# henreedev/audio-pathtracer

Hardware: NVIDIA B200
Metric: bdpt_path_pairs_per_second (higher is better)
Workload: dtype f32 + u64 Q32.32

## Files before the change

audio-pathtracer_b200/csrc/fs_bvh_build.cu:

```cuda
#include "fs_internal.h"
#include <vector>
#include <utility>
#include <stdlib.h>

namespace {

__device__ __forceinline__ uint32_t f2ord(float f)
{
    uint32_t u = __float_as_uint(f);
    return (u & 0x80000000u) ? ~u : (u | 0x80000000u);
}
__host__ __device__ __forceinline__ float ord2f(uint32_t u)
{
    u = (u & 0x80000000u) ? (u & 0x7fffffffu) : ~u;
#if defined(__CUDA_ARCH__)
    return __uint_as_float(u);
#else
    float f; memcpy(&f, &u, 4); return f;
#endif
}

__global__ void k_init_bounds(uint32_t* bounds)
{
    if (threadIdx.x < 3) bounds[threadIdx.x] = 0xffffffffu;
// ... 642 lines not shown
            const int r = c[pick].ref;
            load_children(nodes, r, c[pick], c[k]);
            ++k;
        }
    }
    float lx = c[0].lx, hx = c[0].hx, ly = c[0].ly, hy = c[0].hy, lz = c[0].lz, hz = c[0].hz;
    for (int j = 1; j < k; ++j) {
        lx = fminf(lx, c[j].lx); hx = fmaxf(hx, c[j].hx); ly = fminf(ly, c[j].ly); hy = fmaxf(hy, c[j].hy);
        lz = fminf(lz, c[j].lz); hz = fmaxf(hz, c[j].hz);
    }
    if (!(hx < 1e29f) || !(lx > -1e29f) || !(hy < 1e29f) || !(hz < 1e29f)) {
        hx = fminf(hx, 1e29f); hy = fminf(hy, 1e29f); hz = fminf(hz, 1e29f);
    }
    const float mx = 0.5f * (lx + hx), my = 0.5f * (ly + hy), mz = 0.5f * (lz + hz);
    int slot_of[8], child_in[8];
    for (int j = 0; j < 8; ++j) { slot_of[j] = -1; child_in[j] = -1; }
    for (int it = 0; it < k; ++it) {
        float best = -3.0e38f; int bc = -1, bs = -1;
        for (int j = 0; j < k; ++j) {
            if (slot_of[j] >= 0) continue;
            const float dx = 0.5f * (c[j].lx + c[j].hx) - mx, dy = 0.5f * (c[j].ly + c[j].hy) - my, dz = 0.5f * (c[j].lz + c[j].hz) - mz;
            for (int s = 0; s < 8; ++s) {
                if (child_in[s] >= 0) continue;
                const float cost = ((s & 1) ? dx : -dx) + ((s & 2) ? dy : -dy) + ((s & 4) ? dz : -dz);
                if (cost > best) { best = cost; bc = j; bs = s; }
            }
        }
        slot_of[bc] = bs; child_in[bs] = bc;
    }
    const int ebx = q8_exponent(hx - lx), eby = q8_exponent(hy - ly), ebz = q8_exponent(hz - lz);
    const float ix = __uint_as_float((uint32_t)(254 - ebx) << 23), iy = __uint_as_float((uint32_t)(254 - eby) << 23),
                iz = __uint_as_float((uint32_t)(254 - ebz) << 23);
    uint32_t q[12];
    for (int w = 0; w < 12; ++w) q[w] = 0u;
    uint32_t imask = 0, lmask = 0;
    int refs[8];
    for (int s = 0; s < 8; ++s) {
        const int j = child_in[s];
        uint32_t b[6];
        if (j < 0) { b[0] = b[1] = b[2] = 255u; b[3] = b[4] = b[5] = 0u; refs[s] = W8_EMPTY; }
        else {
            b[0] = q8_lo(c[j].lx, lx, ix); b[1] = q8_lo(c[j].ly, ly, iy); b[2] = q8_lo(c[j].lz, lz, iz);
            b[3] = q8_hi(c[j].hx, lx, ix); b[4] = q8_hi(c[j].hy, ly, iy); b[5] = q8_hi(c[j].hz, lz, iz);
            refs[s] = c[j].ref;
            if (c[j].ref >= 0) imask |= 1u << s; else lmask |= 1u << s;
        }
        for (int a = 0; a < 6; ++a) q[a * 2 + (s >> 2)] |= b[a] << (8 * (s & 3));
    }
    uint4* o = w8tmp + (size_t)i * 5;
    o[0] = make_uint4(__float_as_uint(lx), __float_as_uint(ly), __float_as_uint(lz), ((uint32_t)ebx << 23) | imask | (lmask << 8));
    o[1] = make_uint4((uint32_t)eby << 23, (uint32_t)ebz << 23, 0u, 0u);
    o[2] = make_uint4(q[0], q[1], q[2], q[3]);
    o[3] = make_uint4(q[4], q[5], q[6], q[7]);
    o[4] = make_uint4(q[8], q[9], q[10], q[11]);
    for (int s = 0; s < 8; ++s) w8ref[(size_t)i * 8 + s] = refs[s];
}

__global__ void k_w8_count(const uint4* __restrict__ w8tmp, const int* __restrict__ frontier, uint32_t nf,
                           uint32_t* __restrict__ cnt_in, uint32_t* __restrict__ cnt_leaf)
{
    const uint32_t t = blockIdx.x * blockDim.x + threadIdx.x;
    if (t >= nf) return;
    const uint32_t w = w8tmp[(size_t)frontier[t] * 5].w;
    cnt_in[t] = (uint32_t)__popc(w & 0xffu);
    cnt_leaf[t] = (uint32_t)__popc((w >> 8) & 0xffu);
}

__global__ void k_w8_place(const uint4* __restrict__ w8tmp, const int* __restrict__ w8ref, uint4* __restrict__ dst,
                           const int* __restrict__ frontier, uint32_t nf, const uint32_t* __restrict__ off_in,
                           const uint32_t* __restrict__ off_leaf, uint32_t level_base, uint32_t tri_level_base,
                           int* __restrict__ next_frontier, const float4* __restrict__ tris, float4* __restrict__ tris8,
                           uint32_t* __restrict__ tri8_map)
{
    const uint32_t t = blockIdx.x * blockDim.x + threadIdx.x;
    if (t >= nf) return;
    const int src = frontier[t];
    const uint4* p = w8tmp + (size_t)src * 5;
    uint4* q = dst + (size_t)(level_base + t) * 5;
    uint4 u1 = p[1];
    uint32_t oi = off_in[t], ol = tri_level_base + off_leaf[t];
    u1.z = level_base + nf + oi;
    u1.w = ol;
    q[0] = p[0]; q[1] = u1; q[2] = p[2]; q[3] = p[3]; q[4] = p[4];
    for (int s = 0; s < 8; ++s) {
        const int r = w8ref[(size_t)src * 8 + s];
        if (r == W8_EMPTY) continue;
        if (r >= 0) next_frontier[oi++] = r;
        else {
            const uint32_t first = (uint32_t)(~r) >> 3;
            for (int a = 0; a < 4; ++a) tris8[(size_t)ol * 4 + a] = tris[(size_t)first * 4 + a];
            tri8_map[ol] = first;
            ++ol;
        }
    }
}

__device__ __forceinline__ void store_children(float4* __restrict__ nodes, int i, const cbox& a, const cbox& b)
{
    nodes[(size_t)i * 4] = make_float4(a.lx, a.hx, a.ly, a.hy);
    nodes[(size_t)i * 4 + 1] = make_float4(b.lx, b.hx, b.ly, b.hy);
    nodes[(size_t)i * 4 + 2] = make_float4(a.lz, a.hz, b.lz, b.hz);
    nodes[(size_t)i * 4 + 3] = make_float4(__int_as_float(a.ref), __int_as_float(b.ref), 0.f, 0.f);
}
__device__ __forceinline__ cbox cbox_union(const cbox& a, const cbox& b, int ref)
{
    cbox u;
    u.lx = fminf(a.lx, b.lx); u.hx = fmaxf(a.hx, b.hx); u.ly = fminf(a.ly, b.ly); u.hy = fmaxf(a.hy, b.hy);
    u.lz = fminf(a.lz, b.lz); u.hz = fmaxf(a.hz, b.hz); u.ref = ref; u.src = -1;
    return u;
}

__global__ void k_bvh2_count(const float4* __restrict__ nodes, const int* __restrict__ frontier, uint32_t nf, uint32_t* __restrict__ cnt)
{
    const uint32_t t = blockIdx.x * blockDim.x + threadIdx.x;
    if (t >= nf) return;
    const float4 n3 = nodes[(size_t)frontier[t] * 4 + 3];
    cnt[t] = (__float_as_int(n3.x) >= 0 ? 1u : 0u) + (__float_as_int(n3.y) >= 0 ? 1u : 0u);
}
__global__ void k_bvh2_place(const float4* __restrict__ nodes, const int* __restrict__ frontier, uint32_t nf,
                             const uint32_t* __restrict__ off, int* __restrict__ next)
{
    const uint32_t t = blockIdx.x * blockDim.x + threadIdx.x;
    if (t >= nf) return;
    const float4 n3 = nodes[(size_t)frontier[t] * 4 + 3];
    uint32_t o = off[t];
    const int c0 = __float_as_int(n3.x), c1 = __float_as_int(n3.y);
    if (c0 >= 0) next[o++] = c0;
    if (c1 >= 0) next[o] = c1;
}

__global__ void k_rotate(float4* __restrict__ nodes, const int* __restrict__ level, uint32_t nl, uint32_t* __restrict__ n_done)
{
    const uint32_t t = blockIdx.x * blockDim.x + threadIdx.x;
    if (t >= nl) return;
    const int N = level[t];
    cbox L, R;
    load_children(nodes, N, L, R);
    float best = 0.0f; int op = 0;
    cbox LL, LR, RL, RR;
    if (R.ref >= 0) {
        load_children(nodes, R.ref, RL, RR);
        const float aR = cbox_area(R);
        const float d1 = cbox_area(cbox_union(L, RR, 0)) - aR;
        const float d2 = cbox_area(cbox_union(RL, L, 0)) - aR;
        if (d1 < best) { best = d1; op = 1; }
        if (d2 < best) { best = d2; op = 2; }
    }
    if (L.ref >= 0) {
        load_children(nodes, L.ref, LL, LR);
        const float aL = cbox_area(L);
        const float d3 = cbox_area(cbox_union(R, LR, 0)) - aL;
        const float d4 = cbox_area(cbox_union(LL, R, 0)) - aL;
        if (d3 < best) { best = d3; op = 3; }
        if (d4 < best) { best = d4; op = 4; }
    }
    if (op == 0) return;
    if (op == 1) {
        const cbox Rn = cbox_union(L, RR, R.ref);
        store_children(nodes, R.ref, L, RR);
        store_children(nodes, N, RL, Rn);
    } else if (op == 2) {
        const cbox Rn = cbox_union(RL, L, R.ref);
        store_children(nodes, R.ref, RL, L);
        store_children(nodes, N, RR, Rn);
    } else if (op == 3) {
        const cbox Ln = cbox_union(R, LR, L.ref);
        store_children(nodes, L.ref, R, LR);
        store_children(nodes, N, Ln, LL);
    } else {
        const cbox Ln = cbox_union(LL, R, L.ref);
        store_children(nodes, L.ref, LL, R);
        store_children(nodes, N, Ln, LR);
    }
    atomicAdd(n_done, 1u);
}

__global__ void k_sah_cost(uint32_t n_inner, const float4* __restrict__ nodes, double* __restrict__ out)
{
    const uint32_t i = blockIdx.x * blockDim.x + threadIdx.x;
    double a = 0.0;
    if (i < n_inner) {
        cbox c0, c1;
        load_children(nodes, (int)i, c0, c1);
        a = (double)cbox_area(c0) + (double)cbox_area(c1);
    }
    for (int o = 16; o; o >>= 1) a += __shfl_xor_sync(0xffffffffu, a, o);
    if ((threadIdx.x & 31) == 0 && a != 0.0) atomicAdd(out, a);
}

__device__ __forceinline__ void emit_single(float4 l0, float4 h0, float4* __restrict__ nodes)
{
    float pad = box_pad(l0, h0);
    const float F = 1e30f;
    nodes[0] = make_float4(l0.x - pad, h0.x + pad, l0.y - pad, h0.y + pad);
    nodes[1] = make_float4(F, F, F, F);
    nodes[2] = make_float4(l0.z - pad, h0.z + pad, F, F);
    nodes[3] = make_float4(__int_as_float(~0), __int_as_float(~0), 0.f, 0.f);
}
__global__ void k_emit_single(const float4* __restrict__ bb_lo, const float4* __restrict__ bb_hi,
                              float4* __restrict__ nodes)
{
    emit_single(bb_lo[0], bb_hi[0], nodes);
}

__global__ void k_top_treelet(const float4* __restrict__ nodes, uint32_t n_inner, uint32_t cap,
                              float4* __restrict__ top, uint32_t* __restrict__ n_top_out, int* __restrict__ queue)
{
    if (threadIdx.x != 0 || blockIdx.x != 0) return;
    uint32_t qn = 0;
    queue[qn++] = 0;
    for (uint32_t p = 0; p < qn; ++p) {
        const float4* src = nodes + (size_t)queue[p] * 4;
        float4 n3 = src[3];
        int c0 = __float_as_int(n3.x), c1 = __float_as_int(n3.y);
        if (c0 >= 0 && qn < cap) { queue[qn] = c0; c0 = FS_TOP_FLAG | (int)qn; ++qn; }
        if (c1 >= 0 && qn < cap) { queue[qn] = c1; c1 = FS_TOP_FLAG | (int)qn; ++qn; }
        top[(size_t)p * 4 + 0] = src[0];
        top[(size_t)p * 4 + 1] = src[1];
        top[(size_t)p * 4 + 2] = src[2];
        top[(size_t)p * 4 + 3] = make_float4(__int_as_float(c0), __int_as_float(c1), 0.f, 0.f);
    }
    *n_top_out = qn;
    (void)n_inner;
}

__global__ void k_leaf_stats(int n, const int2* __restrict__ ranges, uint32_t* __restrict__ max_leaf, int leaf_max)
{
    int i = blockIdx.x * blockDim.x + threadIdx.x;
    if (i >= n - 1) return;
    int cnt = ranges[i].y - ranges[i].x + 1;
    if (cnt <= leaf_max) atomicMax(max_leaf, (uint32_t)cnt);
}

__global__ void k_refit_tris(uint32_t n, const float* __restrict__ verts, const uint32_t* __restrict__ tri_orig,
                             const uint32_t* __restrict__ tri_mat, float4* __restrict__ tris, float4* __restrict__ tri_nm)
{
    const uint32_t j = blockIdx.x * blockDim.x + threadIdx.x;
    if (j >= n) return;
    pack_tri(verts, tri_orig[j], tri_mat[j], j, tris, tri_nm);
}

__device__ __forceinline__ void refit_child(int r, const float* __restrict__ verts, const uint32_t* __restrict__ tri_orig,
                                            const float4* ubox, float4& lo, float4& hi)
{
    if (r >= 0) { lo = __ldcg(ubox + 2 * (size_t)r); hi = __ldcg(ubox + 2 * (size_t)r + 1); return; }
    const uint32_t e = (uint32_t)~r, first = e >> 3, cnt = (e & 7u) + 1u;
    tri_box(verts + (size_t)tri_orig[first] * 9, lo, hi);
    for (uint32_t k = 1; k < cnt; ++k) {
        float4 l, h;
        tri_box(verts + (size_t)tri_orig[first + k] * 9, l, h);
        lo = make_float4(fminf(lo.x, l.x), fminf(lo.y, l.y), fminf(lo.z, l.z), 0.f);
        hi = make_float4(fmaxf(hi.x, h.x), fmaxf(hi.y, h.y), fmaxf(hi.z, h.z), 0.f);
    }
}

__global__ void k_refit_nodes(uint32_t n_inner, const float* __restrict__ verts, const uint32_t* __restrict__ tri_orig,
                              const int* __restrict__ parent, const uint32_t* __restrict__ need, uint32_t* __restrict__ arrive,
                              float4* __restrict__ nodes, float4* ubox)
{
    const uint32_t i = blockIdx.x * blockDim.x + threadIdx.x;
    if (i >= n_inner || need[i] != 0u) return;
    int n = (int)i;
    for (;;) {
        const float4 n3 = nodes[(size_t)n * 4 + 3];
        float4 l0, h0, l1, h1;
        refit_child(__float_as_int(n3.x), verts, tri_orig, ubox, l0, h0);
        refit_child(__float_as_int(n3.y), verts, tri_orig, ubox, l1, h1);
        const float p0 = box_pad(l0, h0), p1 = box_pad(l1, h1);
        nodes[(size_t)n * 4 + 0] = make_float4(l0.x - p0, h0.x + p0, l0.y - p0, h0.y + p0);
        nodes[(size_t)n * 4 + 1] = make_float4(l1.x - p1, h1.x + p1, l1.y - p1, h1.y + p1);
        nodes[(size_t)n * 4 + 2] = make_float4(l0.z - p0, h0.z + p0, l1.z - p1, h1.z + p1);
        __stcg(ubox + 2 * (size_t)n, make_float4(fminf(l0.x, l1.x), fminf(l0.y, l1.y), fminf(l0.z, l1.z), 0.f));
        __stcg(ubox + 2 * (size_t)n + 1, make_float4(fmaxf(h0.x, h1.x), fmaxf(h0.y, h1.y), fmaxf(h0.z, h1.z), 0.f));
        __threadfence();
        const int p = parent[n];
        if (p < 0) break;
        if (atomicAdd(arrive + p, 1u) + 1u < need[p]) break;
        __threadfence();
        n = p;
    }
}

__global__ void k_refit_single(const float* __restrict__ verts, const uint32_t* __restrict__ tri_orig, float4* __restrict__ nodes)
{
    float4 lo, hi;
    tri_box(verts + (size_t)tri_orig[0] * 9, lo, hi);
    emit_single(lo, hi, nodes);
}

__global__ void k_requant4(uint32_t n_slots, const float4* __restrict__ nodes, const int* __restrict__ wsrc,
                           const float* __restrict__ grid, uint4* __restrict__ wnodes)
{
    const uint32_t s = blockIdx.x * blockDim.x + threadIdx.x;
    if (s >= n_slots) return;
    const int src = wsrc[s];
    if (src < 0) return;
    cbox a, b;
    load_children(nodes, src >> 1, a, b);
    const cbox& c = (src & 1) ? b : a;
    const uint4 q = quant_box(c.lx, c.hx, c.ly, c.hy, c.lz, c.hz, 0, grid);
    uint4 u = wnodes[s];
    u.x = q.x; u.y = q.y; u.z = q.z;
    wnodes[s] = u;
}

}



#define BCHECK(x) do { cudaError_t e_ = (x); if (e_ != cudaSuccess) { err = e_; goto fail; } } while (0)

static void scan_u32(cudaStream_t st, const uint32_t* in, uint32_t* out, uint32_t n, uint32_t* tile_sums,
                     uint32_t* total, uint64_t* launches)
{
    const uint32_t tiles = (n + SCAN_TILE - 1) / SCAN_TILE;
    k_scan_tiles<<<tiles, SCAN_TILE, 0, st>>>(in, out, n, tile_sums);
    k_sort_scan<<<1, 1024, 0, st>>>(tile_sums, tiles);
    k_scan_add<<<tiles, SCAN_TILE, 0, st>>>(out, n, tile_sums);
    k_scan_total<<<1, 32, 0, st>>>(in, out, n, total);
    *launches += 4;
}

static cudaError_t ploc_build(cudaStream_t st, uint32_t n, const float4* bb_lo, const float4* bb_hi, float4* nodes,
                              uint64_t* launches, int radius)
{
    cudaError_t err = cudaSuccess;
    float4 *lo[2] = {nullptr, nullptr}, *hi[2] = {nullptr, nullptr};
    int* ref[2] = {nullptr, nullptr};
    uint32_t *nn = nullptr, *keep = nullptr, *mflag = nullptr, *keep_scan = nullptr, *merge_scan = nullptr,
             *tile_sums = nullptr, *totals = nullptr;
    const uint32_t n_inner = n - 1;
    const int TPB = 256;
    uint32_t cur = n, made = 0;
    int pp = 0;
    for (int k = 0; k < 2; ++k) {
        BCHECK(cudaMalloc(&lo[k], sizeof(float4) * n));
        BCHECK(cudaMalloc(&hi[k], sizeof(float4) * n));
        BCHECK(cudaMalloc(&ref[k], sizeof(int) * n));
    }
    BCHECK(cudaMalloc(&nn, 4ull * n)); BCHECK(cudaMalloc(&keep, 4ull * n)); BCHECK(cudaMalloc(&mflag, 4ull * n));
    BCHECK(cudaMalloc(&keep_scan, 4ull * n)); BCHECK(cudaMalloc(&merge_scan, 4ull * n));
    BCHECK(cudaMalloc(&tile_sums, 4ull * ((n + SCAN_TILE - 1) / SCAN_TILE + 2)));
    BCHECK(cudaMalloc(&totals, 4 * 2));
    k_ploc_init<<<(n + TPB - 1) / TPB, TPB, 0, st>>>(n, bb_lo, bb_hi, lo[0], hi[0], ref[0]); ++*launches;
    for (int round = 0; cur > 1 && round < 4096; ++round) {
        const uint32_t g = (cur + TPB - 1) / TPB;
        k_ploc_nn<<<g, TPB, 0, st>>>(cur, lo[pp], hi[pp], nn, radius);
        k_ploc_flags<<<g, TPB, 0, st>>>(cur, nn, keep, mflag);
        *launches += 2;
        scan_u32(st, keep, keep_scan, cur, tile_sums, totals, launches);
        scan_u32(st, mflag, merge_scan, cur, tile_sums, totals + 1, launches);
        k_ploc_merge<<<g, TPB, 0, st>>>(cur, nn, keep_scan, merge_scan, keep, mflag, made, n_inner, lo[pp], hi[pp], ref[pp],
                                        lo[pp ^ 1], hi[pp ^ 1], ref[pp ^ 1], nodes);
        ++*launches;
        uint32_t h[2];
        BCHECK(cudaMemcpyAsync(h, totals, sizeof(h), cudaMemcpyDeviceToHost, st));
        BCHECK(cudaStreamSynchronize(st));
        if (h[1] == 0 || h[0] >= cur) { err = cudaErrorUnknown; goto fail; }
        made += h[1];
        cur = h[0];
        pp ^= 1;
    }
    if (cur != 1 || made != n_inner) err = cudaErrorUnknown;
fail:
    for (int k = 0; k < 2; ++k) { cudaFree(lo[k]); cudaFree(hi[k]); cudaFree(ref[k]); }
    cudaFree(nn); cudaFree(keep); cudaFree(mflag); cudaFree(keep_scan); cudaFree(merge_scan); cudaFree(tile_sums); cudaFree(totals);
    return err;
}

static cudaError_t bvh2_rotate(cudaStream_t st, uint32_t n_inner, float4* nodes, int sweeps, uint64_t* launches, uint32_t* n_rot)
{
    cudaError_t err = cudaSuccess;
    int* order = nullptr;
    uint32_t *cnt = nullptr, *off = nullptr, *tile_sums = nullptr, *total = nullptr, *d_done = nullptr;
    const int TPB = 256;
    std::vector<std::pair<uint32_t, uint32_t>> levels;
    const int zero = 0;
    *n_rot = 0;
    BCHECK(cudaMalloc(&order, 4ull * n_inner));
    BCHECK(cudaMalloc(&cnt, 4ull * n_inner)); BCHECK(cudaMalloc(&off, 4ull * n_inner));
    BCHECK(cudaMalloc(&tile_sums, 4ull * ((n_inner + SCAN_TILE - 1) / SCAN_TILE + 2)));
    BCHECK(cudaMalloc(&total, 4)); BCHECK(cudaMalloc(&d_done, 4));
    BCHECK(cudaMemsetAsync(d_done, 0, 4, st));
    for (int sw = 0; sw < sweeps; ++sw) {
        levels.clear();
        BCHECK(cudaMemcpyAsync(order, &zero, 4, cudaMemcpyHostToDevice, st));
        uint32_t base = 0, nf = 1;
        while (nf) {
            levels.push_back(std::make_pair(base, nf));
            const uint32_t g = (nf + TPB - 1) / TPB;
            uint32_t next = 0;
            k_bvh2_count<<<g, TPB, 0, st>>>(nodes, order + base, nf, cnt); ++*launches;
            scan_u32(st, cnt, off, nf, tile_sums, total, launches);
            BCHECK(cudaMemcpyAsync(&next, total, 4, cudaMemcpyDeviceToHost, st));
            BCHECK(cudaStreamSynchronize(st));
            if (base + nf + next > n_inner) { err = cudaErrorUnknown; goto fail; }
            if (next) { k_bvh2_place<<<g, TPB, 0, st>>>(nodes, order + base, nf, off, order + base + nf); ++*launches; }
            base += nf; nf = next;
        }
        for (size_t l = levels.size(); l-- > 0;) {
            const uint32_t nl = levels[l].second;
            k_rotate<<<(nl + TPB - 1) / TPB, TPB, 0, st>>>(nodes, order + levels[l].first, nl, d_done); ++*launches;
        }
    }
    BCHECK(cudaMemcpyAsync(n_rot, d_done, 4, cudaMemcpyDeviceToHost, st));
    BCHECK(cudaStreamSynchronize(st));
    BCHECK(cudaGetLastError());
fail:
    cudaFree(order); cudaFree(cnt); cudaFree(off); cudaFree(tile_sums); cudaFree(total); cudaFree(d_done);
    return err;
}

static cudaError_t wide_compact(cudaStream_t st, uint32_t n_inner, const uint4* sparse, const int* sparse_prov, uint4** dense_out,
                                int** dense_prov_out, uint32_t* n_wide_out, uint64_t* launches)
{
    cudaError_t err = cudaSuccess;
    int* fr[2] = {nullptr, nullptr};
    uint32_t *cnt = nullptr, *off = nullptr, *tile_sums = nullptr, *total = nullptr;
    uint4* dense = nullptr;
    int* dense_prov = nullptr;
    const int TPB = 256;
    uint32_t nf = 1, base = 0;
    int pp = 0;
    const int zero = 0;
    BCHECK(cudaMalloc(&fr[0], 4ull * n_inner)); BCHECK(cudaMalloc(&fr[1], 4ull * n_inner));
    BCHECK(cudaMalloc(&cnt, 4ull * n_inner)); BCHECK(cudaMalloc(&off, 4ull * n_inner));
    BCHECK(cudaMalloc(&tile_sums, 4ull * ((n_inner + SCAN_TILE - 1) / SCAN_TILE + 2)));
    BCHECK(cudaMalloc(&total, 4));
    BCHECK(cudaMalloc(&dense, sizeof(uint4) * 4ull * n_inner));
    BCHECK(cudaMalloc(&dense_prov, sizeof(int) * 4ull * n_inner));
    BCHECK(cudaMemcpyAsync(fr[0], &zero, 4, cudaMemcpyHostToDevice, st));
    while (nf) {
        const uint32_t g = (nf + TPB - 1) / TPB;
        uint32_t next = 0;
        k_wide_count<<<g, TPB, 0, st>>>(sparse, fr[pp], nf, cnt); ++*launches;
        scan_u32(st, cnt, off, nf, tile_sums, total, launches);
        k_wide_place<<<g, TPB, 0, st>>>(sparse, dense, sparse_prov, dense_prov, fr[pp], nf, off, base, fr[pp ^ 1]); ++*launches;
        BCHECK(cudaMemcpyAsync(&next, total, 4, cudaMemcpyDeviceToHost, st));
        BCHECK(cudaStreamSynchronize(st));
        base += nf; nf = next; pp ^= 1;
        if (base + nf > n_inner) { err = cudaErrorUnknown; goto fail; }
    }
    BCHECK(cudaGetLastError());
    *dense_out = dense; dense = nullptr; *dense_prov_out = dense_prov; dense_prov = nullptr; *n_wide_out = base;
fail:
    cudaFree(fr[0]); cudaFree(fr[1]); cudaFree(cnt); cudaFree(off); cudaFree(tile_sums); cudaFree(total); cudaFree(dense); cudaFree(dense_prov);
    return err;
}

static cudaError_t w8_build(cudaStream_t st, uint32_t n, uint32_t n_inner, const float4* nodes, const float4* tris,
                            fs_bvh_device* out, uint64_t* launches, bool dp)
{
    cudaError_t err = cudaSuccess;
    float* T = nullptr; int* parent = nullptr; uint32_t *need = nullptr, *arrive = nullptr;
    uint4 *tmp = nullptr, *dense = nullptr, *fit = nullptr;
    int *ref = nullptr, *fr[2] = {nullptr, nullptr};
    uint32_t *cnt_in = nullptr, *cnt_leaf = nullptr, *off_in = nullptr, *off_leaf = nullptr, *tile_sums = nullptr, *total = nullptr;
    float4* tris8 = nullptr; uint32_t* map = nullptr;
    const int TPB = 256;
    uint32_t nf = 1, base = 0, tri_base = 0;
    int pp = 0;
    const int zero = 0;
    BCHECK(cudaMalloc(&tmp, sizeof(uint4) * 5ull * n_inner));
    BCHECK(cudaMalloc(&ref, 4ull * 8 * n_inner));
    BCHECK(cudaMalloc(&dense, sizeof(uint4) * 5ull * n_inner));
    BCHECK(cudaMalloc(&fr[0], 4ull * n_inner)); BCHECK(cudaMalloc(&fr[1], 4ull * n_inner));
    BCHECK(cudaMalloc(&cnt_in, 4ull * n_inner)); BCHECK(cudaMalloc(&cnt_leaf, 4ull * n_inner));
    BCHECK(cudaMalloc(&off_in, 4ull * n_inner)); BCHECK(cudaMalloc(&off_leaf, 4ull * n_inner));
    BCHECK(cudaMalloc(&tile_sums, 4ull * ((n_inner + SCAN_TILE - 1) / SCAN_TILE + 2)));
    BCHECK(cudaMalloc(&total, 8));
    BCHECK(cudaMalloc(&tris8, sizeof(float4) * 4ull * n));
    BCHECK(cudaMalloc(&map, 4ull * n));
    if (dp) {
        BCHECK(cudaMalloc(&T, sizeof(float) * 8ull * n_inner));
        BCHECK(cudaMalloc(&parent, 4ull * n_inner)); BCHECK(cudaMalloc(&need, 4ull * n_inner)); BCHECK(cudaMalloc(&arrive, 4ull * n_inner));
        BCHECK(cudaMemsetAsync(arrive, 0, 4ull * n_inner, st));
        k_w8_parents<<<(n_inner + TPB - 1) / TPB, TPB, 0, st>>>(n_inner, nodes, parent, need);
        k_wide_dp<8><<<(n_inner + TPB - 1) / TPB, TPB, 0, st>>>(n_inner, nodes, parent, need, arrive, T);
        *launches += 2;
    }
    k_emit8<<<(n_inner + TPB - 1) / TPB, TPB, 0, st>>>(n_inner, nodes, T, tmp, ref); ++*launches;
    BCHECK(cudaMemcpyAsync(fr[0], &zero, 4, cudaMemcpyHostToDevice, st));
    while (nf) {
        const uint32_t g = (nf + TPB - 1) / TPB;
        uint32_t next[2] = {0, 0};
        k_w8_count<<<g, TPB, 0, st>>>(tmp, fr[pp], nf, cnt_in, cnt_leaf); ++*launches;
        scan_u32(st, cnt_in, off_in, nf, tile_sums, total, launches);
        scan_u32(st, cnt_leaf, off_leaf, nf, tile_sums, total + 1, launches);
        k_w8_place<<<g, TPB, 0, st>>>(tmp, ref, dense, fr[pp], nf, off_in, off_leaf, base, tri_base, fr[pp ^ 1], tris, tris8, map);
        ++*launches;
        BCHECK(cudaMemcpyAsync(next, total, 8, cudaMemcpyDeviceToHost, st));
        BCHECK(cudaStreamSynchronize(st));
        base += nf; nf = next[0]; tri_base += next[1]; pp ^= 1;
        if ((uint64_t)base + nf > n_inner || tri_base > n) { err = cudaErrorUnknown; goto fail; }
    }
    BCHECK(cudaGetLastError());
    if (tri_base != n) { err = cudaErrorUnknown; goto fail; }
    BCHECK(cudaMalloc(&fit, sizeof(uint4) * 5ull * base));
    BCHECK(cudaMemcpyAsync(fit, dense, sizeof(uint4) * 5ull * base, cudaMemcpyDeviceToDevice, st));
    BCHECK(cudaStreamSynchronize(st));
    out->w8nodes = fit; fit = nullptr; out->n_w8 = base;
    out->tris8 = tris8; tris8 = nullptr; out->tri8_map = map; map = nullptr;
fail:
    cudaFree(T); cudaFree(parent); cudaFree(need); cudaFree(arrive);
    cudaFree(tmp); cudaFree(ref); cudaFree(dense); cudaFree(fit); cudaFree(fr[0]); cudaFree(fr[1]); cudaFree(cnt_in); cudaFree(cnt_leaf);
    cudaFree(off_in); cudaFree(off_leaf); cudaFree(tile_sums); cudaFree(total); cudaFree(tris8); cudaFree(map);
    return err;
}

cudaError_t fs_bvh_build(cudaStream_t st, const float* d_verts, const uint32_t* d_mats, uint64_t T64,
                         fs_bvh_device* out, uint64_t* launches, uint32_t leaf_max_u, uint32_t builder, uint32_t collapse_u)
{
    const int leaf_max = (int)(leaf_max_u < 1 ? 1 : (leaf_max_u > 8 ? 8 : leaf_max_u));
    const int collapse = (int)collapse_u;
    cudaError_t err = cudaSuccess;
    const uint32_t n = (uint32_t)T64;
    fs_bvh_free(out);
    out->n_tris = n;
    if (n == 0) return cudaSuccess;
    const uint32_t n_inner = n > 1 ? n - 1 : 1;
    const uint32_t n_blocks_sort = (n + SORT_TILE - 1) / SORT_TILE;
    float4 *tlo = nullptr, *thi = nullptr, *bb_lo = nullptr, *bb_hi = nullptr;
    uint64_t *keys0 = nullptr, *keys1 = nullptr;
    uint32_t *vals0 = nullptr, *vals1 = nullptr, *block_hist = nullptr, *misc = nullptr, *arrive = nullptr;
    float* grid = nullptr;
    int2 *children = nullptr, *ranges = nullptr;
    int *parent = nullptr, *queue = nullptr;
    const int TPB = 256;
    const uint32_t gb = (n + TPB - 1) / TPB;

    BCHECK(cudaMalloc(&tlo, sizeof(float4) * n));
    BCHECK(cudaMalloc(&thi, sizeof(float4) * n));
    BCHECK(cudaMalloc(&bb_lo, sizeof(float4) * (2ull * n)));
    BCHECK(cudaMalloc(&bb_hi, sizeof(float4) * (2ull * n)));
    BCHECK(cudaMalloc(&keys0, 8ull * n));
    BCHECK(cudaMalloc(&keys1, 8ull * n));
    BCHECK(cudaMalloc(&vals0, 4ull * n));
    BCHECK(cudaMalloc(&vals1, 4ull * n));
    BCHECK(cudaMalloc(&block_hist, 4ull * 256 * n_blocks_sort));
    BCHECK(cudaMalloc(&misc, 4 * 16));
    BCHECK(cudaMalloc(&arrive, 4ull * n_inner));
    BCHECK(cudaMalloc(&children, sizeof(int2) * n_inner));
    BCHECK(cudaMalloc(&ranges, sizeof(int2) * n_inner));
    BCHECK(cudaMalloc(&parent, 4ull * 2 * n));
    BCHECK(cudaMalloc(&queue, 4ull * FS_TOP_CAP));
    BCHECK(cudaMalloc(&out->nodes, sizeof(float4) * 4ull * n_inner));
    BCHECK(cudaMalloc(&out->wnodes, sizeof(uint4) * 4ull * n_inner));
    BCHECK(cudaMalloc(&out->wsrc, sizeof(int) * 4ull * n_inner));
    BCHECK(cudaMalloc(&grid, sizeof(float) * 8));
    BCHECK(cudaMalloc(&out->tris, sizeof(float4) * 4ull * n));
    BCHECK(cudaMalloc(&out->tri_orig, 4ull * n));
    BCHECK(cudaMalloc(&out->tri_mat, 4ull * n));
    BCHECK(cudaMalloc(&out->tri_nm, sizeof(float4) * (size_t)n));
    BCHECK(cudaMalloc(&out->top_nodes, sizeof(float4) * 4ull * FS_TOP_CAP));
    out->n_inner = n_inner;

    BCHECK(cudaMemsetAsync(misc, 0, 4 * 16, st));
    BCHECK(cudaMemsetAsync(arrive, 0, 4ull * n_inner, st));
    k_init_bounds<<<1, 32, 0, st>>>(misc); ++*launches;
    k_tri_bounds<<<gb, TPB, 0, st>>>(d_verts, n, tlo, thi, misc, misc + 6); ++*launches;
    k_morton<<<gb, TPB, 0, st>>>(tlo, thi, n, misc, keys0, vals0); ++*launches;
    {
        uint64_t *ki = keys0, *ko = keys1;
        uint32_t *vi = vals0, *vo = vals1;
        for (int pass = 0; pass < 8; ++pass) {
            int shift = pass * 8;
            k_sort_hist<<<n_blocks_sort, SORT_THREADS, 0, st>>>(ki, n, shift, block_hist, n_blocks_sort);
            k_sort_scan<<<1, 1024, 0, st>>>(block_hist, 256u * n_blocks_sort);
            k_sort_scatter<<<n_blocks_sort, SORT_THREADS, 0, st>>>(ki, vi, ko, vo, n, shift, block_hist, n_blocks_sort);
            *launches += 3;
            uint64_t* tk = ki; ki = ko; ko = tk;
            uint32_t* tv = vi; vi = vo; vo = tv;
        }
    }
    k_pack<<<gb, TPB, 0, st>>>(d_verts, d_mats, vals0, n, tlo, thi, out->tris, out->tri_orig, out->tri_mat, out->tri_nm, bb_lo, bb_hi);
    ++*launches;
    if (n == 1) {
        k_emit_single<<<1, 1, 0, st>>>(bb_lo, bb_hi, out->nodes); ++*launches;
        out->max_leaf = 1;
    } else if (builder == 1 && n >= 3) {
        int cand[4] = {5, 10, 24, 64}, n_cand = 4;
        if (const char* e = getenv("FS_TUNE_PLOC_R")) { int v = atoi(e); if (v >= 1 && v <= 256) { cand[0] = v; n_cand = 1; } }
        if (n < 4096) n_cand = 1;
        double best_cost = 0.0; int best = -1;
        float4* alt = nullptr; double* d_cost = nullptr;
        float* cT4 = nullptr; int* cpar = nullptr; uint32_t *cneed = nullptr, *carr = nullptr;
        if (n_cand > 1) { BCHECK(cudaMalloc(&alt, sizeof(float4) * 4ull * n_inner)); BCHECK(cudaMalloc(&d_cost, 8)); }
        for (int ci = 0; ci < n_cand; ++ci) {
            float4* dst = (n_cand > 1) ? alt : out->nodes;
            BCHECK(ploc_build(st, n, bb_lo, bb_hi, dst, launches, cand[ci]));
            if (n_cand == 1) break;
            double h_cost = 0.0;
            BCHECK(cudaMemsetAsync(d_cost, 0, 8, st));
            k_sah_cost<<<(n_inner + TPB - 1) / TPB, TPB, 0, st>>>(n_inner, dst, d_cost); ++*launches;
            BCHECK(cudaMemcpyAsync(&h_cost, d_cost, 8, cudaMemcpyDeviceToHost, st));
            BCHECK(cudaStreamSynchronize(st));
            if (getenv("FS_VERBOSE")) fprintf(stderr, "[frequensee] PLOC radius %d: surface-area cost %.6g\n", cand[ci], h_cost);
            if (collapse & 16) {
                if (!cT4) {
                    BCHECK(cudaMalloc(&cT4, sizeof(float) * 4ull * n_inner)); BCHECK(cudaMalloc(&cpar, 4ull * n_inner));
                    BCHECK(cudaMalloc(&cneed, 4ull * n_inner)); BCHECK(cudaMalloc(&carr, 4ull * n_inner));
                }
                float root_cost = 0.f;
                BCHECK(cudaMemsetAsync(carr, 0, 4ull * n_inner, st));
                k_w8_parents<<<(n_inner + TPB - 1) / TPB, TPB, 0, st>>>(n_inner, dst, cpar, cneed);
                k_wide_dp<4><<<(n_inner + TPB - 1) / TPB, TPB, 0, st>>>(n_inner, dst, cpar, cneed, carr, cT4);
                *launches += 2;
                BCHECK(cudaMemcpyAsync(&root_cost, cT4, 4, cudaMemcpyDeviceToHost, st));
                BCHECK(cudaStreamSynchronize(st));
                if (getenv("FS_VERBOSE")) fprintf(stderr, "[frequensee] PLOC radius %d: summed area of the 4-wide nodes %.6g\n", cand[ci], (double)root_cost);
                h_cost = (double)root_cost;
            }
            if (best < 0 || h_cost < best_cost) {
                best = ci; best_cost = h_cost;
                BCHECK(cudaMemcpyAsync(out->nodes, alt, sizeof(float4) * 4ull * n_inner, cudaMemcpyDeviceToDevice, st));
            }
        }
        if (alt) { cudaStreamSynchronize(st); cudaFree(alt); cudaFree(d_cost); }
        cudaFree(cT4); cudaFree(cpar); cudaFree(cneed); cudaFree(carr);
        out->max_leaf = 1;
        {
            int sweeps = 0;
            if (const char* e = getenv("FS_TUNE_ROTATE")) { int v = atoi(e); if (v >= 0 && v <= 64) sweeps = v; }
            if (sweeps && n >= 4096) {
                uint32_t n_rot = 0;
                BCHECK(bvh2_rotate(st, n_inner, out->nodes, sweeps, launches, &n_rot));
                if (getenv("FS_VERBOSE")) {
                    double* d_c = nullptr; double h_c = 0.0;
                    if (cudaMalloc(&d_c, 8) == cudaSuccess) {
                        cudaMemsetAsync(d_c, 0, 8, st);
                        k_sah_cost<<<(n_inner + TPB - 1) / TPB, TPB, 0, st>>>(n_inner, out->nodes, d_c);
                        cudaMemcpyAsync(&h_c, d_c, 8, cudaMemcpyDeviceToHost, st); cudaStreamSynchronize(st); cudaFree(d_c);
                    }
                    fprintf(stderr, "[frequensee] %d rotation sweeps: %u rotations, surface-area cost %.6g\n", sweeps, n_rot, h_c);
                }
            }
        }
    } else {
        k_karras<<<gb, TPB, 0, st>>>(keys0, (int)n, children, ranges, parent); ++*launches;
        k_refit<<<gb, TPB, 0, st>>>((int)n, children, parent, bb_lo, bb_hi, arrive); ++*launches;
        k_emit<<<gb, TPB, 0, st>>>((int)n, children, ranges, bb_lo, bb_hi, out->nodes, leaf_max); ++*launches;
        k_leaf_stats<<<gb, TPB, 0, st>>>((int)n, ranges, misc + 8, leaf_max); ++*launches;
    }
    k_quant_grid<<<1, 32, 0, st>>>(out->nodes, grid); ++*launches;
    if ((collapse & 16) && n >= 3) {
        float* T4 = nullptr; int* par = nullptr; uint32_t *need = nullptr, *arr = nullptr;
        cudaError_t e4 = cudaSuccess;
        if ((e4 = cudaMalloc(&T4, sizeof(float) * 4ull * n_inner)) == cudaSuccess && (e4 = cudaMalloc(&par, 4ull * n_inner)) == cudaSuccess &&
            (e4 = cudaMalloc(&need, 4ull * n_inner)) == cudaSuccess && (e4 = cudaMalloc(&arr, 4ull * n_inner)) == cudaSuccess &&
            (e4 = cudaMemsetAsync(arr, 0, 4ull * n_inner, st)) == cudaSuccess) {
            k_w8_parents<<<(n_inner + TPB - 1) / TPB, TPB, 0, st>>>(n_inner, out->nodes, par, need);
            k_wide_dp<4><<<(n_inner + TPB - 1) / TPB, TPB, 0, st>>>(n_inner, out->nodes, par, need, arr, T4);
            k_emit4_dp<<<(n_inner + TPB - 1) / TPB, TPB, 0, st>>>(n_inner, out->nodes, T4, grid, out->wnodes, out->wsrc);
            *launches += 3;
            e4 = cudaStreamSynchronize(st);
        }
        cudaFree(T4); cudaFree(par); cudaFree(need); cudaFree(arr);
        BCHECK(e4);
    } else {
        k_emit4<<<(n_inner + TPB - 1) / TPB, TPB, 0, st>>>(n_inner, out->nodes, grid, out->wnodes, out->wsrc, collapse & 1); ++*launches;
    }
    out->n_wide = n_inner;
    if (!(collapse & 2)) {
        uint4* dense = nullptr; int* dense_prov = nullptr; uint32_t n_wide = 0;
        BCHECK(wide_compact(st, n_inner, out->wnodes, out->wsrc, &dense, &dense_prov, &n_wide, launches));
        cudaFree(out->wnodes); out->wnodes = dense; out->n_wide = n_wide;
        cudaFree(out->wsrc); out->wsrc = dense_prov;
    }
    {
        cudaResourceDesc rd; memset(&rd, 0, sizeof(rd));
        rd.resType = cudaResourceTypeLinear;
        rd.res.linear.devPtr = out->nodes;
        rd.res.linear.desc = cudaCreateChannelDesc<float4>();
        rd.res.linear.sizeInBytes = sizeof(float4) * 4ull * n_inner;
        cudaTextureDesc td; memset(&td, 0, sizeof(td));
        td.readMode = cudaReadModeElementType;
        if (cudaCreateTextureObject(&out->nodes_tex, &rd, &td, nullptr) != cudaSuccess) { out->nodes_tex = 0; (void)cudaGetLastError(); }
        rd.res.linear.devPtr = out->tris;
        rd.res.linear.sizeInBytes = sizeof(float4) * 4ull * n;
        if (cudaCreateTextureObject(&out->tris_tex, &rd, &td, nullptr) != cudaSuccess) { out->tris_tex = 0; (void)cudaGetLastError(); }
        rd.res.linear.devPtr = out->wnodes;
        rd.res.linear.desc = cudaCreateChannelDesc<uint4>();
        rd.res.linear.sizeInBytes = sizeof(uint4) * 4ull * out->n_wide;
        if (cudaCreateTextureObject(&out->wnodes_tex, &rd, &td, nullptr) != cudaSuccess) { out->wnodes_tex = 0; (void)cudaGetLastError(); }
    }
    k_top_treelet<<<1, 32, 0, st>>>(out->nodes, n_inner, FS_TOP_CAP, out->top_nodes, misc + 7, queue); ++*launches;
    BCHECK(cudaGetLastError());
    if (builder == 1 && n >= 3 && out->max_leaf == 1 && (collapse & 4)) BCHECK(w8_build(st, n, n_inner, out->nodes, out->tris, out, launches, !(collapse & 8)));
    {
        uint32_t h[16];
        BCHECK(cudaMemcpyAsync(h, misc, sizeof(h), cudaMemcpyDeviceToHost, st));
        BCHECK(cudaStreamSynchronize(st));
        out->n_top = h[7];
        if (n > 1 && !(builder == 1 && n >= 3)) out->max_leaf = h[8] ? h[8] : 1;
        out->extent = ord2f(h[6]);
        float hg[6];
        BCHECK(cudaMemcpy(hg, grid, sizeof(hg), cudaMemcpyDeviceToHost));
        for (int a = 0; a < 3; ++a) { out->qbase[a] = hg[a]; out->qscale[a] = hg[3 + a]; }
    }
fail:
    cudaFree(tlo); cudaFree(thi); cudaFree(bb_lo); cudaFree(bb_hi); cudaFree(keys0); cudaFree(keys1);
    cudaFree(vals0); cudaFree(vals1); cudaFree(block_hist); cudaFree(misc); cudaFree(arrive);
    cudaFree(children); cudaFree(ranges); cudaFree(parent); cudaFree(queue); cudaFree(grid);
    if (err != cudaSuccess) fs_bvh_free(out);
    return err;
}

void fs_bvh_free(fs_bvh_device* b)
{
    if (b->nodes_tex) cudaDestroyTextureObject(b->nodes_tex);
    if (b->tris_tex) cudaDestroyTextureObject(b->tris_tex);
    if (b->wnodes_tex) cudaDestroyTextureObject(b->wnodes_tex);
    cudaFree(b->w8nodes); cudaFree(b->tris8); cudaFree(b->tri8_map);
    cudaFree(b->nodes); cudaFree(b->wnodes); cudaFree(b->tris); cudaFree(b->tri_orig); cudaFree(b->tri_mat); cudaFree(b->tri_nm); cudaFree(b->top_nodes);
    cudaFree(b->wsrc);
    cudaFree(b->rf.parent); cudaFree(b->rf.need); cudaFree(b->rf.arrive); cudaFree(b->rf.ubox); cudaFree(b->rf.queue); cudaFree(b->rf.misc);
    memset(b, 0, sizeof(*b));
}

cudaError_t fs_bvh_refit(cudaStream_t st, const float* d_verts, fs_bvh_device* b, uint64_t* launches, float* cost_ratio)
{
    cudaError_t err = cudaSuccess;
    const uint32_t n = b->n_tris, n_inner = b->n_inner;
    const int TPB = 256;
    fs_bvh_device::refit_scratch& r = b->rf;
    struct { double cost[2]; float grid[8]; uint32_t n_top; } h;
    if (cost_ratio) *cost_ratio = 1.0f;
    if (n == 0) return cudaSuccess;
    if (!r.misc) {
        BCHECK(cudaMalloc(&r.parent, 4ull * n_inner));
        BCHECK(cudaMalloc(&r.need, 4ull * n_inner));
        BCHECK(cudaMalloc(&r.arrive, 4ull * n_inner));
        BCHECK(cudaMalloc(&r.ubox, sizeof(float4) * 2ull * n_inner));
        BCHECK(cudaMalloc(&r.queue, 4ull * FS_TOP_CAP));
        BCHECK(cudaMalloc(&r.misc, sizeof(h)));
        BCHECK(cudaMemsetAsync(r.parent, 0xff, 4ull * n_inner, st));
        BCHECK(cudaMemsetAsync(r.misc, 0, sizeof(h), st));
        k_w8_parents<<<(n_inner + TPB - 1) / TPB, TPB, 0, st>>>(n_inner, b->nodes, r.parent, r.need);
        k_sah_cost<<<(n_inner + TPB - 1) / TPB, TPB, 0, st>>>(n_inner, b->nodes, (double*)r.misc);
        *launches += 2;
        BCHECK(cudaMemcpyAsync(&r.cost0, r.misc, sizeof(double), cudaMemcpyDeviceToHost, st));
    }
    BCHECK(cudaMemsetAsync(r.arrive, 0, 4ull * n_inner, st));
    BCHECK(cudaMemsetAsync((double*)r.misc + 1, 0, sizeof(double), st));
    k_refit_tris<<<(n + TPB - 1) / TPB, TPB, 0, st>>>(n, d_verts, b->tri_orig, b->tri_mat, b->tris, b->tri_nm);
    if (n == 1) k_refit_single<<<1, 1, 0, st>>>(d_verts, b->tri_orig, b->nodes);
    else k_refit_nodes<<<(n_inner + TPB - 1) / TPB, TPB, 0, st>>>(n_inner, d_verts, b->tri_orig, r.parent, r.need, r.arrive, b->nodes, r.ubox);
    k_sah_cost<<<(n_inner + TPB - 1) / TPB, TPB, 0, st>>>(n_inner, b->nodes, (double*)r.misc + 1);
    {
        float* d_grid = (float*)((char*)r.misc + offsetof(decltype(h), grid));
        k_quant_grid<<<1, 32, 0, st>>>(b->nodes, d_grid);
        const uint32_t n_slots = 4u * b->n_wide;
        k_requant4<<<(n_slots + TPB - 1) / TPB, TPB, 0, st>>>(n_slots, b->nodes, b->wsrc, d_grid, b->wnodes);
        k_top_treelet<<<1, 32, 0, st>>>(b->nodes, n_inner, FS_TOP_CAP, b->top_nodes,
                                        (uint32_t*)((char*)r.misc + offsetof(decltype(h), n_top)), r.queue);
    }
    *launches += 6;
    BCHECK(cudaGetLastError());
    BCHECK(cudaMemcpyAsync(&h, r.misc, sizeof(h), cudaMemcpyDeviceToHost, st));
    BCHECK(cudaStreamSynchronize(st));
    for (int a = 0; a < 3; ++a) { b->qbase[a] = h.grid[a]; b->qscale[a] = h.grid[3 + a]; }
    b->n_top = h.n_top;
    if (cost_ratio) *cost_ratio = r.cost0 > 0.0 ? (float)(h.cost[1] / r.cost0) : 1.0f;
fail:
    return err;
}
```

Baseline: 246.9 million.

## Add parallel SAH-driven subtree reinsertion pass to BVH2 build

Adds an iterative GPU reinsertion optimizer for the binary BVH after PLOC build. Each iteration searches, for large-area nodes, a better insertion slot by branch-and-bound on surface-area cost, resolves conflicts with atomicMax locks along ancestor paths, applies the moves, refits, and rolls back if SAH cost rises. The aim is to lower traversal cost in the path tracer, paid for with extra build time made of many launches and a host sync per iteration.

After: 262.1 million (median of 6 runs). +6.2%, better.

```diff
diff --git a/audio-pathtracer_b200/csrc/fs_bvh_build.cu b/audio-pathtracer_b200/csrc/fs_bvh_build.cu
--- a/audio-pathtracer_b200/csrc/fs_bvh_build.cu
+++ b/audio-pathtracer_b200/csrc/fs_bvh_build.cu
@@ -968,6 +968,143 @@
     uint4 u = wnodes[s];
     u.x = q.x; u.y = q.y; u.z = q.z;
     wnodes[s] = u;
+}
+
+#ifndef FS_REINSERT_ITERS
+#define FS_REINSERT_ITERS 32
+#endif
+constexpr int RI_MAXD = 64;
+constexpr int RI_STACK = 128;
+
+__device__ __forceinline__ cbox slot_box(const float4* __restrict__ nodes, int slot)
+{
+    cbox a, b;
+    load_children(nodes, slot >> 1, a, b);
+    return (slot & 1) ? b : a;
+}
+__device__ __forceinline__ int slot_ref(const float4* nodes, int slot)
+{
+    return ((const int*)(nodes + (size_t)(slot >> 1) * 4 + 3))[slot & 1];
+}
+
+__global__ void k_ri_hist(uint32_t n_inner, const float4* __restrict__ nodes, uint32_t* __restrict__ hist)
+{
+    const uint32_t s = blockIdx.x * blockDim.x + threadIdx.x + 2u;
+    if (s >= 2u * n_inner) return;
+    atomicAdd(hist + (f2ord(cbox_area(slot_box(nodes, (int)s))) >> 20), 1u);
+}
+
+__global__ void k_ri_search(uint32_t n_inner, const float4* __restrict__ nodes, const int* __restrict__ parent, float thr,
+                            float min_gain, float* __restrict__ mv_gain, int* __restrict__ mv_dst)
+{
+    const int s = (int)(blockIdx.x * blockDim.x + threadIdx.x) + 2;
+    if (s >= 2 * (int)n_inner) return;
+    mv_dst[s] = -1;
+    const int P = s >> 1;
+    cbox a, b;
+    load_children(nodes, P, a, b);
+    const cbox N = (s & 1) ? b : a, S = (s & 1) ? a : b;
+    const float aN = cbox_area(N);
+    if (!(aN >= thr)) return;
+    struct ent { int slot; float c, g; };
+    ent st[RI_STACK];
+    int sp = 0;
+    cbox cur = S;
+    float g = 0.0f;
+    for (int c = P, d = 0;; ++d) {
+        const int u = parent[c];
+        if (u < 0) break;
+        if (d == RI_MAXD) return;
+        cbox l, r;
+        load_children(nodes, u, l, r);
+        const int cs = (l.ref == c) ? 0 : 1;
+        const cbox& cb = cs ? r : l;
+        const cbox& ob = cs ? l : r;
+        g += (c == P) ? cbox_area(cb) : cbox_area(cb) - cbox_area(cur);
+        cur = cbox_union(cur, ob, 0);
+        st[sp++] = ent{2 * u + (cs ^ 1), 0.0f, g};
+        c = u;
+    }
+    for (int i = 0, j = sp - 1; i < j; ++i, --j) { const ent t = st[i]; st[i] = st[j]; st[j] = t; }
+    if (S.ref >= 0) {
+        const float c0 = cbox_area(cbox_union(S, N, 0)) - cbox_area(S), aP = st[sp - 1].g;
+        st[sp++] = ent{2 * S.ref, c0, aP};
+        st[sp++] = ent{2 * S.ref + 1, c0, aP};
+    }
+    float best = -min_gain * aN; int bdst = -1;
+    while (sp) {
+        const ent e = st[--sp];
+        if (e.c + aN - e.g >= best) continue;
+        const cbox X = slot_box(nodes, e.slot);
+        const float u = cbox_area(cbox_union(X, N, 0));
+        const float tot = e.c + u - e.g;
+        if (tot < best) { best = tot; bdst = e.slot; }
+        if (X.ref >= 0) {
+            const float c2 = e.c + u - cbox_area(X);
+            if (c2 + aN - e.g < best && sp + 2 <= RI_STACK) {
+                st[sp++] = ent{2 * X.ref + 1, c2, e.g};
+                st[sp++] = ent{2 * X.ref, c2, e.g};
+            }
+        }
+    }
+    mv_gain[s] = -best;
+    mv_dst[s] = bdst;
+}
+
+template <typename F>
+__device__ __forceinline__ void ri_lockset(const int* __restrict__ parent, int s, int dst, F f)
+{
+    int up[RI_MAXD + 2]; int d = 0;
+    for (int c = s >> 1; c >= 0 && d < RI_MAXD + 2; c = parent[c]) up[d++] = c;
+    int lca = 0;
+    for (int v = dst >> 1; v >= 0; v = parent[v]) {
+        bool on = false;
+        for (int k = 0; k < d; ++k) if (up[k] == v) { on = true; break; }
+        if (on) { lca = v; break; }
+        f(v);
+    }
+    for (int k = 0; k < d; ++k) { f(up[k]); if (up[k] == lca) break; }
+    if (d > 1) f(up[1]);
+}
+
+__device__ __forceinline__ unsigned long long ri_key(float gain, int s)
+{
+    return ((unsigned long long)__float_as_uint(gain) << 32) | (unsigned long long)(uint32_t)s;
+}
+
+__global__ void k_ri_lock(uint32_t n_inner, const int* __restrict__ parent, const float* __restrict__ mv_gain,
+                          const int* __restrict__ mv_dst, unsigned long long* __restrict__ lock)
+{
+    const int s = (int)(blockIdx.x * blockDim.x + threadIdx.x) + 2;
+    if (s >= 2 * (int)n_inner || mv_dst[s] < 0) return;
+    const unsigned long long key = ri_key(mv_gain[s], s);
+    ri_lockset(parent, s, mv_dst[s], [&](int v) { atomicMax(lock + v, key); });
+}
+
+__device__ __forceinline__ void set_ref(float4* nodes, int slot, int ref)
+{
+    ((int*)(nodes + (size_t)(slot >> 1) * 4 + 3))[slot & 1] = ref;
+}
+
+__global__ void k_ri_apply(uint32_t n_inner, const int* __restrict__ parent, const float* __restrict__ mv_gain,
+                           const int* __restrict__ mv_dst, const unsigned long long* __restrict__ lock, float4* nodes,
+                           uint32_t* __restrict__ n_moved)
+{
+    const int s = (int)(blockIdx.x * blockDim.x + threadIdx.x) + 2;
+    if (s >= 2 * (int)n_inner) return;
+    const int dst = mv_dst[s];
+    if (dst < 0) return;
+    const unsigned long long key = ri_key(mv_gain[s], s);
+    bool own = true;
+    ri_lockset(parent, s, dst, [&](int v) { own = own && (lock[v] == key); });
+    if (!own) return;
+    const int P = s >> 1, G = parent[P];
+    const int Nr = slot_ref(nodes, s), Sr = slot_ref(nodes, s ^ 1), Xr = slot_ref(nodes, dst);
+    set_ref(nodes, 2 * G + (slot_ref(nodes, 2 * G) == P ? 0 : 1), Sr);
+    set_ref(nodes, dst, P);
+    set_ref(nodes, 2 * P, Nr);
+    set_ref(nodes, 2 * P + 1, Xr);
+    atomicAdd(n_moved, 1u);
 }
 
 }
@@ -1074,6 +1211,81 @@
     BCHECK(cudaGetLastError());
 fail:
     cudaFree(order); cudaFree(cnt); cudaFree(off); cudaFree(tile_sums); cudaFree(total); cudaFree(d_done);
+    return err;
+}
+
+static cudaError_t bvh2_reinsert(cudaStream_t st, uint32_t n_inner, const float* d_verts, const uint32_t* tri_orig,
+                                 float4* nodes, int iters, uint64_t* launches)
+{
+    cudaError_t err = cudaSuccess;
+    int *parent = nullptr, *mv_dst = nullptr;
+    uint32_t *need = nullptr, *arrive = nullptr, *hist = nullptr;
+    float4 *ubox = nullptr, *backup = nullptr;
+    float* mv_gain = nullptr;
+    unsigned long long* lock = nullptr;
+    char* misc = nullptr;
+    const int TPB = 256;
+    const uint32_t n_slots = 2u * n_inner - 2u, gs = (n_slots + TPB - 1) / TPB, gi = (n_inner + TPB - 1) / TPB;
+    std::vector<uint32_t> h_hist(4096);
+    double cost0 = 0.0, prev = 0.0;
+    int it = 0;
+    uint32_t total_moves = 0;
+    float thr = 0.0f;
+    BCHECK(cudaMalloc(&parent, 4ull * n_inner)); BCHECK(cudaMalloc(&need, 4ull * n_inner)); BCHECK(cudaMalloc(&arrive, 4ull * n_inner));
+    BCHECK(cudaMalloc(&ubox, sizeof(float4) * 2ull * n_inner)); BCHECK(cudaMalloc(&backup, sizeof(float4) * 4ull * n_inner));
+    BCHECK(cudaMalloc(&lock, 8ull * n_inner));
+    BCHECK(cudaMalloc(&mv_gain, 4ull * 2 * n_inner)); BCHECK(cudaMalloc(&mv_dst, 4ull * 2 * n_inner));
+    BCHECK(cudaMalloc(&hist, 4ull * 4096)); BCHECK(cudaMalloc(&misc, 16));
+    BCHECK(cudaMemsetAsync(hist, 0, 4ull * 4096, st));
+    BCHECK(cudaMemsetAsync(misc, 0, 16, st));
+    k_ri_hist<<<gs, TPB, 0, st>>>(n_inner, nodes, hist);
+    k_sah_cost<<<gi, TPB, 0, st>>>(n_inner, nodes, (double*)misc);
+    *launches += 2;
+    BCHECK(cudaMemcpyAsync(h_hist.data(), hist, 4ull * 4096, cudaMemcpyDeviceToHost, st));
+    BCHECK(cudaMemcpyAsync(&cost0, misc, 8, cudaMemcpyDeviceToHost, st));
+    BCHECK(cudaStreamSynchronize(st));
+    {
+        uint64_t acc = 0;
+        for (int bin = 4095; bin >= 0; --bin) {
+            acc += h_hist[bin];
+            if (acc * 10 >= n_slots) { thr = ord2f((uint32_t)bin << 20); break; }
+        }
+    }
+    prev = cost0;
+    for (it = 0; it < iters; ++it) {
+        struct { double cost; uint32_t moved; } h;
+        BCHECK(cudaMemsetAsync(lock, 0, 8ull * n_inner, st));
+        BCHECK(cudaMemsetAsync(misc, 0, 16, st));
+        k_w8_parents<<<gi, TPB, 0, st>>>(n_inner, nodes, parent, need);
+        k_ri_search<<<gs, TPB, 0, st>>>(n_inner, nodes, parent, thr, 1e-5f, mv_gain, mv_dst);
+        k_ri_lock<<<gs, TPB, 0, st>>>(n_inner, parent, mv_gain, mv_dst, lock);
+        BCHECK(cudaMemcpyAsync(backup, nodes, sizeof(float4) * 4ull * n_inner, cudaMemcpyDeviceToDevice, st));
+        k_ri_apply<<<gs, TPB, 0, st>>>(n_inner, parent, mv_gain, mv_dst, lock, nodes, (uint32_t*)(misc + 8));
+        BCHECK(cudaMemsetAsync(arrive, 0, 4ull * n_inner, st));
+        k_w8_parents<<<gi, TPB, 0, st>>>(n_inner, nodes, parent, need);
+        k_refit_nodes<<<gi, TPB, 0, st>>>(n_inner, d_verts, tri_orig, parent, need, arrive, nodes, ubox);
+        k_sah_cost<<<gi, TPB, 0, st>>>(n_inner, nodes, (double*)misc);
+        *launches += 7;
+        BCHECK(cudaMemcpyAsync(&h, misc, sizeof(h), cudaMemcpyDeviceToHost, st));
+        BCHECK(cudaStreamSynchronize(st));
+        BCHECK(cudaGetLastError());
+        if (h.moved == 0) break;
+        if (h.cost > prev) {
+            BCHECK(cudaMemcpyAsync(nodes, backup, sizeof(float4) * 4ull * n_inner, cudaMemcpyDeviceToDevice, st));
+            BCHECK(cudaStreamSynchronize(st));
+            break;
+        }
+        total_moves += h.moved;
+        const bool small = prev - h.cost < 1e-4 * prev;
+        prev = h.cost;
+        if (small) { ++it; break; }
+    }
+    if (getenv("FS_VERBOSE"))
+        fprintf(stderr, "[frequensee] reinsertion: %d iterations, %u moves, surface-area cost %.6g -> %.6g (%.2f %%)\n", it,
+                total_moves, cost0, prev, cost0 > 0.0 ? 100.0 * (prev - cost0) / cost0 : 0.0);
+fail:
+    cudaFree(parent); cudaFree(need); cudaFree(arrive); cudaFree(ubox); cudaFree(backup); cudaFree(lock);
+    cudaFree(mv_gain); cudaFree(mv_dst); cudaFree(hist); cudaFree(misc);
     return err;
 }
 
@@ -1302,6 +1514,11 @@
                 }
             }
         }
+        {
+            int iters = FS_REINSERT_ITERS;
+            if (const char* e = getenv("FS_TUNE_REINSERT")) { int v = atoi(e); if (v >= 0 && v <= 256) iters = v; }
+            if (iters && n >= 4096) BCHECK(bvh2_reinsert(st, n_inner, d_verts, out->tri_orig, out->nodes, iters, launches));
+        }
     } else {
         k_karras<<<gb, TPB, 0, st>>>(keys0, (int)n, children, ranges, parent); ++*launches;
         k_refit<<<gb, TPB, 0, st>>>((int)n, children, parent, bb_lo, bb_hi, arrive); ++*launches;
```
